# okian/kofft

Measured on AMD Instinct MI355X. Metric: batched 4096-pt c32 FFT throughput, GPoints/s (achieved HBM GB/s: roofline.achieved), higher is better.
Workload: dtype f32

## Files before the change

include/kofft_hip.h:

```cpp
#ifndef KOFFT_HIP_H
#define KOFFT_HIP_H

#include <stddef.h>
#include <stdint.h>

#ifdef __cplusplus
extern "C" {
#endif

#define KOFFT_OK 0
#define KOFFT_ERR_EMPTY_INPUT 1
#define KOFFT_ERR_NON_POWER_OF_TWO_NO_STD 2
#define KOFFT_ERR_MISMATCHED_LENGTHS 3
#define KOFFT_ERR_INVALID_STRIDE 4
#define KOFFT_ERR_INVALID_HOP_SIZE 5
#define KOFFT_ERR_INVALID_VALUE 6
#define KOFFT_ERR_HIP (-1)
#define KOFFT_ERR_UNSUPPORTED (-2)
#define KOFFT_ERR_NULL (-3)
#define KOFFT_ERR_ALLOC (-4)
#define KOFFT_ERR_RCCL (-5)

typedef struct kofft_hip_ctx kofft_hip_ctx;

// ... 198 lines not shown
                                         int mode, float level, int cmap, int depth, int scale, int layout, const uint32_t *pix_of_bin,
                                         void *d_out);
int kofft_hip_set_spectrogram_transpose(kofft_hip_ctx *ctx, int on);
int kofft_hip_stft_picture_f32(kofft_hip_ctx *ctx, const float *signal, size_t rows, size_t len, size_t row_stride, const float *window,
                               size_t win_len, size_t hop, size_t frames, int max_mode, const float *max_in, float *max_out, int mode,
                               float level, int cmap, int depth, int channels, int scale, int layout, const uint32_t *pix_of_bin, void *out);
int kofft_hip_dev_stft_picture_f32(kofft_hip_ctx *ctx, const float *d_signal, size_t rows, size_t len, size_t row_stride,
                                   const float *d_window, size_t win_len, size_t hop, size_t frames, int max_mode, const float *d_max_in,
                                   float *d_max_out, int mode, float level, int cmap, int depth, int channels, int scale, int layout,
                                   const uint32_t *pix_of_bin, void *d_out);
int kofft_hip_log_bin_map(size_t bins, uint32_t *pix_of_bin);
int kofft_hip_map_color_u8(float t, int cmap, unsigned char *rgb);

int kofft_hip_dct_direct_f32(kofft_hip_ctx *ctx, int type, const float *in, float *out, size_t n, size_t batch);
int kofft_hip_dct_direct_f32_dev(kofft_hip_ctx *ctx, int type, const float *d_in, float *d_out, size_t n, size_t batch);
int kofft_hip_dst_direct_f32(kofft_hip_ctx *ctx, int type, const float *in, float *out, size_t n, size_t batch);
int kofft_hip_dst_direct_f32_dev(kofft_hip_ctx *ctx, int type, const float *d_in, float *d_out, size_t n, size_t batch);
int kofft_hip_set_direct_tiled(kofft_hip_ctx *ctx, int on);
int kofft_hip_set_persist_claim_pct(kofft_hip_ctx *ctx, int pct);
int kofft_hip_persist_claim_debug(kofft_hip_ctx *ctx, unsigned out[9]);
int kofft_hip_set_persist_walk(kofft_hip_ctx *ctx, int mode);
int kofft_hip_set_persist_keep_bytes(kofft_hip_ctx *ctx, size_t bytes);
int kofft_hip_persist_walk_debug(kofft_hip_ctx *ctx, unsigned long long out[4]);
int kofft_hip_dct_direct_table_f32(int type, size_t n, float *C);
int kofft_hip_dst_direct_table_f32(int type, size_t n, float *C);
int kofft_hip_dst_planner_table_f32(int type, size_t n, float *out);
int kofft_hip_dst_planner_table_f64(int type, size_t n, double *out);

int kofft_hip_czt_f32(kofft_hip_ctx *ctx, const float *in, float *out, size_t n, size_t m, float wr, float wi, float ar, float ai,
                      size_t batch);
int kofft_hip_dev_czt_f32(kofft_hip_ctx *ctx, const float *d_in, float *d_out, size_t n, size_t m, float wr, float wi, float ar, float ai,
                          size_t batch);
int kofft_hip_goertzel_f32(kofft_hip_ctx *ctx, const float *in, float *out, size_t n, size_t batch, float sample_rate,
                           const float *target_freqs, size_t nfreq);
int kofft_hip_dev_goertzel_f32(kofft_hip_ctx *ctx, const float *d_in, float *d_out, size_t n, size_t batch, float sample_rate,
                               const float *target_freqs, size_t nfreq);
int kofft_hip_set_czt_route(kofft_hip_ctx *ctx, int mode);
int kofft_hip_czt_table_f32(size_t n, size_t m, float wr, float wi, float ar, float ai, float *C);
int kofft_hip_goertzel_coeff_f32(size_t n, float sample_rate, const float *target_freqs, size_t nfreq, float *coeff);

int kofft_hip_dht_f32(kofft_hip_ctx *ctx, const float *in, float *out, size_t n, size_t batch);
int kofft_hip_dev_dht_f32(kofft_hip_ctx *ctx, const float *d_in, float *d_out, size_t n, size_t batch);
int kofft_hip_set_dht_table_device(kofft_hip_ctx *ctx, int on);
int kofft_hip_dht_table_f32(size_t n, float *H);
int kofft_hip_libm_trigf(const float *x, size_t count, float *cos_out, float *sin_out);

// ... 136 lines not shown
```

kofft_amd/_lib.py:

```python
from __future__ import annotations

import ctypes as C
import os
import re
from pathlib import Path

_PKG = Path(__file__).resolve().parent
LIB_PATH = _PKG / "lib" / "libkofft_hip.so"
HEADER_PATH = _PKG.parent / "include" / "kofft_hip.h"


class LibraryMissing(RuntimeError):
    pass


_c_f = C.POINTER(C.c_float)
_c_d = C.POINTER(C.c_double)
_sz = C.c_size_t
_ctx = C.c_void_p

SIGNATURES = {
    "kofft_hip_strerror": (C.c_char_p, [C.c_int]),
    "kofft_hip_last_error": (C.c_char_p, [_ctx]),
    "kofft_hip_version": (C.c_char_p, []),
# ... 105 lines not shown
    "kofft_hip_db_scale_f32": (C.c_int, [_ctx, C.c_void_p, _sz, C.c_void_p, C.c_float, C.c_void_p]),
    "kofft_hip_dev_db_scale_f32": (C.c_int, [_ctx, C.c_void_p, _sz, C.c_void_p, C.c_float, C.c_void_p]),
    "kofft_hip_spectrogram_render_f32": (C.c_int, [_ctx, C.c_void_p, _sz, _sz, C.c_void_p, C.c_int, C.c_float, C.c_int, C.c_int, C.c_int, C.c_int,
                                                   C.c_void_p, C.c_void_p]),
    "kofft_hip_dev_spectrogram_render_f32": (C.c_int, [_ctx, C.c_void_p, _sz, _sz, C.c_void_p, C.c_int, C.c_float, C.c_int, C.c_int, C.c_int, C.c_int,
                                                       C.c_void_p, C.c_void_p]),
    "kofft_hip_set_spectrogram_transpose": (C.c_int, [_ctx, C.c_int]),
    "kofft_hip_stft_picture_f32": (C.c_int, [_ctx, C.c_void_p, _sz, _sz, _sz, C.c_void_p, _sz, _sz, _sz, C.c_int, C.c_void_p, C.c_void_p, C.c_int,
                                             C.c_float, C.c_int, C.c_int, C.c_int, C.c_int, C.c_int, C.c_void_p, C.c_void_p]),
    "kofft_hip_dev_stft_picture_f32": (C.c_int, [_ctx, C.c_void_p, _sz, _sz, _sz, C.c_void_p, _sz, _sz, _sz, C.c_int, C.c_void_p, C.c_void_p, C.c_int,
                                                 C.c_float, C.c_int, C.c_int, C.c_int, C.c_int, C.c_int, C.c_void_p, C.c_void_p]),
    "kofft_hip_log_bin_map": (C.c_int, [_sz, C.c_void_p]),
    "kofft_hip_map_color_u8": (C.c_int, [C.c_float, C.c_int, C.c_void_p]),
    "kofft_hip_dct_direct_f32": (C.c_int, [_ctx, C.c_int, C.c_void_p, C.c_void_p, _sz, _sz]),
    "kofft_hip_dct_direct_f32_dev": (C.c_int, [_ctx, C.c_int, C.c_void_p, C.c_void_p, _sz, _sz]),
    "kofft_hip_dst_direct_f32": (C.c_int, [_ctx, C.c_int, C.c_void_p, C.c_void_p, _sz, _sz]),
    "kofft_hip_dst_direct_f32_dev": (C.c_int, [_ctx, C.c_int, C.c_void_p, C.c_void_p, _sz, _sz]),
    "kofft_hip_set_direct_tiled": (C.c_int, [_ctx, C.c_int]),
    "kofft_hip_set_persist_claim_pct": (C.c_int, [_ctx, C.c_int]),
    "kofft_hip_persist_claim_debug": (C.c_int, [_ctx, C.c_void_p]),
    "kofft_hip_set_persist_walk": (C.c_int, [_ctx, C.c_int]),
    "kofft_hip_set_persist_keep_bytes": (C.c_int, [_ctx, C.c_size_t]),
    "kofft_hip_persist_walk_debug": (C.c_int, [_ctx, C.c_void_p]),
    "kofft_hip_dct_direct_table_f32": (C.c_int, [C.c_int, _sz, C.c_void_p]),
    "kofft_hip_dst_direct_table_f32": (C.c_int, [C.c_int, _sz, C.c_void_p]),
    "kofft_hip_dst_planner_table_f32": (C.c_int, [C.c_int, _sz, C.c_void_p]),
    "kofft_hip_dst_planner_table_f64": (C.c_int, [C.c_int, _sz, C.c_void_p]),
    "kofft_hip_czt_f32": (C.c_int, [_ctx, C.c_void_p, C.c_void_p, _sz, _sz, C.c_float, C.c_float, C.c_float, C.c_float, _sz]),
    "kofft_hip_dev_czt_f32": (C.c_int, [_ctx, C.c_void_p, C.c_void_p, _sz, _sz, C.c_float, C.c_float, C.c_float, C.c_float, _sz]),
    "kofft_hip_goertzel_f32": (C.c_int, [_ctx, C.c_void_p, C.c_void_p, _sz, _sz, C.c_float, C.c_void_p, _sz]),
    "kofft_hip_dev_goertzel_f32": (C.c_int, [_ctx, C.c_void_p, C.c_void_p, _sz, _sz, C.c_float, C.c_void_p, _sz]),
    "kofft_hip_set_czt_route": (C.c_int, [_ctx, C.c_int]),
    "kofft_hip_czt_table_f32": (C.c_int, [_sz, _sz, C.c_float, C.c_float, C.c_float, C.c_float, C.c_void_p]),
    "kofft_hip_dht_f32": (C.c_int, [_ctx, C.c_void_p, C.c_void_p, _sz, _sz]),
    "kofft_hip_dev_dht_f32": (C.c_int, [_ctx, C.c_void_p, C.c_void_p, _sz, _sz]),
    "kofft_hip_set_dht_table_device": (C.c_int, [_ctx, C.c_int]),
    "kofft_hip_dht_table_f32": (C.c_int, [_sz, C.c_void_p]),
    "kofft_hip_libm_trigf": (C.c_int, [C.c_void_p, _sz, C.c_void_p, C.c_void_p]),
    "kofft_hip_window_f32": (C.c_int, [C.c_int, _sz, C.c_float, C.c_void_p]),
    "kofft_hip_goertzel_coeff_f32": (C.c_int, [_sz, C.c_float, C.c_void_p, _sz, C.c_void_p]),
    "kofft_hip_dwt_f32": (C.c_int, [_ctx, C.c_int, C.c_void_p, C.c_void_p, C.c_void_p, _sz, _sz]),
    "kofft_hip_dwt_f32_dev": (C.c_int, [_ctx, C.c_int, C.c_void_p, C.c_void_p, C.c_void_p, _sz, _sz]),
    "kofft_hip_idwt_f32": (C.c_int, [_ctx, C.c_int, C.c_void_p, C.c_void_p, C.c_void_p, _sz, _sz]),
    "kofft_hip_idwt_f32_dev": (C.c_int, [_ctx, C.c_int, C.c_void_p, C.c_void_p, C.c_void_p, _sz, _sz]),
    "kofft_hip_dwt_multi_f32": (C.c_int, [_ctx, C.c_int, C.c_void_p, C.c_void_p, C.c_void_p, _sz, _sz, _sz]),
    "kofft_hip_dwt_multi_f32_dev": (C.c_int, [_ctx, C.c_int, C.c_void_p, C.c_void_p, C.c_void_p, _sz, _sz, _sz]),
# ... 88 lines not shown
```

kofft_amd/api.py:

```python
from __future__ import annotations

import ctypes as C
import os
import enum
from typing import Optional, Sequence

import numpy as np

from . import _lib


class FftError(Exception):

    EmptyInput = 1
    NonPowerOfTwoNoStd = 2
    MismatchedLengths = 3
    InvalidStride = 4
    InvalidHopSize = 5
    InvalidValue = 6
    _names = {1: "EmptyInput", 2: "NonPowerOfTwoNoStd", 3: "MismatchedLengths", 4: "InvalidStride",
              5: "InvalidHopSize", 6: "InvalidValue"}

    def __init__(self, code: int):
        self.code = int(code)
# ... 993 lines not shown
            raise TypeError("the Hartley transform is f32-only, like the reference (hartley.rs)")
        a = self._rbuf(x)
        if a.ndim != 2:
            raise TypeError("dht_batch expects a 2-D [batch, n] array")
        out = np.empty(a.shape, np.float32)
        self._check(self._lib.kofft_hip_dht_f32(self._ctx, _ptr(a), _ptr(out), a.shape[1], a.shape[0]))
        return out

    def dht_dev(self, d_in: int, d_out: int, n: int, batch: int) -> None:
        if min(int(n), int(batch)) < 0:
            raise ValueError("n and batch are usize in the reference: they cannot be negative")
        self._check(self._lib.kofft_hip_dev_dht_f32(self._ctx, C.c_void_p(d_in), C.c_void_p(d_out), int(n), int(batch)))

    def set_dht_table_device(self, on: bool) -> None:
        self._check(self._lib.kofft_hip_set_dht_table_device(self._ctx, int(bool(on))))

    def set_persist_claim_pct(self, pct: int) -> None:
        self._check(self._lib.kofft_hip_set_persist_claim_pct(self._ctx, int(pct)))

    def set_persist_walk(self, mode: int, keep_bytes: int | None = None) -> None:
        self._check(self._lib.kofft_hip_set_persist_walk(self._ctx, int(mode)))
        if keep_bytes is not None:
            self._check(self._lib.kofft_hip_set_persist_keep_bytes(self._ctx, int(keep_bytes)))

    def set_czt_route(self, mode: int) -> None:
        self._check(self._lib.kofft_hip_set_czt_route(self._ctx, int(mode)))

    def _spectral_in(self, x, what: str):
        if self.dtype != np.float32:
            raise TypeError(f"{what} is f32-only, like the reference ({what}.rs)")
        dev = hasattr(x, "data_ptr") and hasattr(x, "is_cuda")
        if dev:
            import torch

            if not x.is_cuda or x.dtype != torch.float32:
                raise TypeError(f"{what}: a torch input must be a float32 tensor on the device")
            a = x.contiguous()
        else:
            a = np.ascontiguousarray(x, np.float32)
        if a.ndim not in (1, 2):
            raise TypeError(f"{what} expects a 1-D signal or a 2-D [batch, n] array")
        return (a.reshape(1, -1) if a.ndim == 1 else a), a.ndim == 1, dev

    def czt(self, x, m: int, w, a):
        rows, one, dev = self._spectral_in(x, "czt")
        if int(m) < 0:
# ... 1302 lines not shown
```

kofft_amd/csrc/fft_persist.hip.h:

```cpp
#pragma once

#include "fft_wg.hip.h"

namespace kofft {

template <typename T, int L, int S0, int Q>
__device__ __forceinline__ void load_pass_twiddles(cpx<T> *twr, const int k, const cpx<T> *__restrict__ tw)
{
#pragma unroll
    for (int t = 0; t < Q; ++t) {
#pragma unroll
        for (int h = 0; h < (1 << t); ++h) {
            const int idx = (k << (L - 1 - S0 - t)) + (bitrev(h, t) << (L - 1 - t));
            twr[(1 << t) - 1 + h] = tw[idx];
        }
    }
}

template <typename T, int Q>
__device__ __forceinline__ void reg_pass_r(cpx<T> *v, const cpx<T> *twr)
{
#pragma unroll
    for (int t = 0; t < Q; ++t) {
        const int pos = Q - 1 - t;
// ... 82 lines not shown
template <class CFG, class = void>
struct persist_depth { static constexpr int value = 1; };
template <class CFG>
struct persist_depth<CFG, decltype((void)CFG::DEPTH)> { static constexpr int value = CFG::DEPTH; };

template <class CFG, class = void>
struct persist_tw_global { static constexpr bool value = false; };
template <class CFG>
struct persist_tw_global<CFG, decltype((void)CFG::kTwGlobal)> { static constexpr bool value = CFG::kTwGlobal; };

template <class CFG, class = void>
struct persist_claim { static constexpr bool value = false; };
template <class CFG>
struct persist_claim<CFG, decltype((void)CFG::kClaim)> { static constexpr bool value = CFG::kClaim; };

constexpr unsigned kPersistClaimShards = 2, kPersistClaimMaxShards = 8, kPersistClaimLine = 128 / sizeof(unsigned);
static_assert(kPersistClaimShards >= 1 && kPersistClaimShards <= kPersistClaimMaxShards, "claim words");
constexpr size_t kPersistClaimBytes = (kPersistClaimMaxShards + 1) * 128;
struct PersistClaim {
    unsigned *counters;
    size_t split;
    size_t keep_from;
    unsigned mirror;
};
constexpr unsigned long long kPersistClaimEmpty = ~0ull;
template <class IO>
struct PersistClaimIO : IO {
    PersistClaim claim;
};
struct NoXchg {
    static constexpr bool keep = false;
    __device__ __forceinline__ void put() const {}
    __device__ __forceinline__ void get() const {}
};

template <typename T, int L, int RL, int EPI, class IO, class CFG>
struct PersistState {
    static constexpr int R = 1 << RL;
    static constexpr int NP = (L + RL - 1) / RL;
    static constexpr bool TWG = persist_tw_global<CFG>::value;
    static constexpr bool TW1_REG = !TWG && !(NP == 2 && CFG::kTwLastInLds);
    static constexpr bool TW2_REG = !TWG && NP >= 3 && !(CFG::kTwLastInLds && NP == 3);
    static constexpr bool TW3_REG = !TWG && NP >= 4 && !CFG::kTwLastInLds;
    cpx<T> tw1[TW1_REG ? R - 1 : 1], tw2[TW2_REG ? R - 1 : 1], tw3[TW3_REG ? R - 1 : 1];
    typename IO::Inv inv[CFG::kInvInLds ? 1 : R];
    const typename IO::Inv *inv_lds;
    const cpx<T> *tw_lds;
    const cpx<T> *rt_lds;
    int g1, g2, g3, sc;
};

template <class IO, int TPT, bool PAIR = io_pairs_in_wave<IO>::value>
struct persist_raw {
    using type = typename IO::Raw;
    static constexpr int extra = 0;
    static constexpr bool pair = false, pair_lds = false;
};
// ... 178 lines not shown
            constexpr int NK = R / 2;
            cpx<T> kept[NK];
            int ki = 0;
#pragma unroll
            for (int u = 0; u < R; ++u)
                if (LastG::out_index(0, u) < N / 2) kept[ki++] = cur[u];
            float m[NK];
            const float top = IO::template mags_of<NK>(kept, m);
            ki = 0;
#pragma unroll
            for (int u = 0; u < R; ++u)
                if (LastG::out_index(0, u) < N / 2) io.store_d_mag(od, lane_bytes, LastG::out_index(0, u), m[ki++], row_off);
            if constexpr (io_row_acc<IO>::value) io.acc_row(xf0, active ? top : 0.0f);
            else if (active) acc = __builtin_fmaxf(acc, top);
        } else if constexpr (io_half_keep<IO>::value) {
            static_assert((LastG::out_index(0, 1) % TPT) == 0 && TPT <= N / 2, "register part and thread part of the index: disjoint bit fields");
#pragma unroll
            for (int u = 0; u < R; ++u) {
                if (LastG::out_index(0, u) < N / 2) io.store_d_kept(od, lane_bytes, LastG::out_index(0, u), cur[u], row_off);
                else if (LastG::out_index(0, u) == N / 2) io.store_d_nyquist(od, tau, LastG::out_index(0, u), cur[u], row_off);
            }
        } else {
        if constexpr (persist_claim<CFG>::value) {
            if (xchg.keep) {
#pragma unroll
                for (int u = 0; u < R; ++u) io.template store_d<AUX_DEFAULT>(od, lane_bytes, LastG::out_index(0, u), cur[u], row_off);
            } else {
#pragma unroll
                for (int u = 0; u < R; ++u) io.template store_d<kStoreAux>(od, lane_bytes, LastG::out_index(0, u), cur[u], row_off);
            }
        } else {
#pragma unroll
        for (int u = 0; u < R; ++u) {
            if constexpr (io_has_acc<IO>::value) io.store_d_acc(od, lane_bytes, LastG::out_index(0, u), cur[u], row_off, acc);
            else io.store_d(od, lane_bytes, LastG::out_index(0, u), cur[u], row_off);
        }
        }
        }
    }
}

template <typename T, int L, int RL, int EPI, class IO, class CFG>
__global__ __launch_bounds__(CFG::BLOCK, CFG::MINW) void fft_persist_kernel(const IO io, const cpx<T> *__restrict__ tw,
                                                                            const size_t batch)
{
    constexpr int BLOCK = CFG::BLOCK, NBUF = CFG::NBUF;
    constexpr int N = 1 << L;
// ... 126 lines not shown
        return;
    }

    constexpr int DEPTH = persist_depth<CFG>::value;
    static_assert(DEPTH == 1 || DEPTH == 2, "prefetch distance");
    Raw ra[RS], rb[RS];
    const int in_lane_bytes = tau * IO::kRawBytes;
    const int in_row_off = (G == 1) ? 0 : sub * (int)io.in_slot_bytes();
    auto group_cnt = [&](size_t b) -> int {
        const size_t first = b + wslot;
        return first >= batch ? 0 : (batch - first < (size_t)G ? (int)(batch - first) : G);
    };
    auto issue = [&](Raw *dst, const size_t b) {
        const rsrc_t d = io.in_desc_n(mem_row(b) + wslot, group_cnt(b));
        if constexpr (RawSel::pair || RawSel::pair_lds) {
#pragma unroll
            for (int u = 0; u < R; ++u) dst[u] = io.fetch_pair_d(d, in_lane_bytes, FirstG::in_index(0, u), in_row_off);
            dst[R] = io.fetch_last_d(d, in_row_off);
        } else {
#pragma unroll
            for (int u = 0; u < R; ++u) dst[u] = io.fetch_d(d, in_lane_bytes, FirstG::in_index(0, u), in_row_off);
        }
    };
    issue(ra, base);
    typename persist_acc<IO>::type acc{};
    if constexpr (io_has_acc<IO>::value) acc = io.acc_init();
    auto finish = [&]() {
        if constexpr (io_has_acc<IO>::value) io.acc_finish(acc);
        if constexpr (CLAIMS) claim_leave();
    };

    if constexpr (CLAIMS) {
        struct ClaimXchg {
            unsigned long long *word;
            size_t first;
            unsigned len;
            const unsigned *ticket;
            size_t *claimed;
            bool writer;
            bool keep;
            __device__ __forceinline__ void put() const
            {
                if (writer) {
                    const unsigned off = XPB * *ticket;
                    *word = off < len ? first + off : kPersistClaimEmpty;
                }
            }
            __device__ __forceinline__ void get() const { *claimed = *word; }
        };
        auto claim_walk_on = [&]() -> size_t {
            if (tid == 0) {
                ++claim_exhausted;
                claim_shard = (claim_shard + 1) % kPersistClaimShards;
                claim_word[1] = claim_now();
            }
            __syncthreads();
            return claim_word[1];
        };
#define KOFFT_PERSIST_STEP_CLAIM(CUR, NXT, LEAVE)                                                                    \
    {                                                                                                                \
        const bool more = nbase < batch;                                                      \
        const bool walked = nbase + step < io.claim.split;                                    \
        const bool claims = more && !walked && tid == 0;                                                             \
        unsigned ticket;  \
        size_t claimed = batch;                                                                                      \
        if (claims) ticket = atomicAdd(claim_counter(claim_shard), 1u);                                              \
        __builtin_amdgcn_sched_barrier(0);                                   \
        issue(NXT, nbase);                                                                                           \
        __builtin_amdgcn_sched_barrier(0);                           \
        const ClaimXchg xchg{claim_word, io.claim.split + (size_t)claim_shard * claim_piece, claim_len(claim_shard), &ticket, &claimed, claims, \
                             __builtin_amdgcn_readfirstlane((unsigned)(base >= io.claim.keep_from)) != 0u}; \
        persist_transform<T, L, RL, EPI, CFG>(CUR, st, io, tw, buf0, buf1, mem_row(base) + wslot, group_cnt(base), sub, tau, acc, NoPrefetchParts{}, xchg); \
        if (!more) LEAVE;                                                                                            \
         \
        if (!walked && __builtin_amdgcn_readfirstlane((unsigned)(claimed >> 32)) == ~0u) claimed = claim_walk_on();   \
        base = nbase;                                                                                                \
        nbase = walked ? nbase + step : (size_t)claimed;                         \
    }
        KOFFT_PERSIST_STEP_CLAIM(ra, rb, { finish(); return; })
        for (;;) {
            KOFFT_PERSIST_STEP_CLAIM(rb, ra, break)
            KOFFT_PERSIST_STEP_CLAIM(ra, rb, break)
        }
        finish();
#undef KOFFT_PERSIST_STEP_CLAIM
    } else if constexpr (DEPTH == 1 && St::TWG && !(RawSel::pair || RawSel::pair_lds)) {
        constexpr bool TOP = persist_twg_top_part(L);
        constexpr int PARTS = TOP ? NP : NP - 1;
#define KOFFT_PERSIST_STEP_PARTS(CUR, NXT, LEAVE)                                                                    \
    {                                                                                                                \
        const size_t nbase = base + step;                                                                            \
        const bool more = nbase < batch;                                                      \
        const rsrc_t nd = io.in_desc_n(nbase + wslot, group_cnt(nbase));                                             \
        auto part = [&](const int i) {                                                                               \
            _Pragma("unroll") for (int u = 0; u < R; ++u)                                                            \
                if (u * PARTS / R == i) NXT[u] = io.fetch_d(nd, in_lane_bytes, FirstG::in_index(0, u), in_row_off);  \
        };                                                                                                           \
        if constexpr (TOP) {                                                                                         \
            part(0);                                                                                                 \
            __builtin_amdgcn_sched_barrier(0);                                                                       \
        }                                                                                                            \
        persist_transform<T, L, RL, EPI, CFG>(CUR, st, io, tw, buf0, buf1, base + wslot, group_cnt(base), sub, tau, acc, part); \
        if (!more) LEAVE;                                                                                            \
        base = nbase;                                                                                                \
    }
        KOFFT_PERSIST_STEP_PARTS(ra, rb, { finish(); return; })
        for (;;) {
// ... 49 lines not shown
```

kofft_amd/csrc/fft_wg.hip.h:

```cpp
#pragma once

#include "fft_device.hip.h"

namespace kofft {

__host__ __device__ constexpr int lds_pad(int i) { return i + (i >> 4); }
__host__ __device__ constexpr int lds_elems(int n) { return n + (n >> 4) + 1; }


struct NoInv {};

template <class IO, class = void>
struct io_has_acc { static constexpr bool value = false; };
template <class IO>
struct io_has_acc<IO, decltype((void)IO::kHasAcc)> { static constexpr bool value = IO::kHasAcc; };
template <class IO, class = void>
struct io_frame_rem { static constexpr bool value = false; };
template <class IO>
struct io_frame_rem<IO, decltype((void)IO::kFrameRem)> { static constexpr bool value = IO::kFrameRem; };
template <class IO, class = void>
struct io_half_spectrum { static constexpr bool value = false; };
template <class IO>
struct io_half_spectrum<IO, decltype((void)IO::kHalfSpectrum)> { static constexpr bool value = IO::kHalfSpectrum; };

// ... 38 lines not shown
    __device__ __forceinline__ Raw fetch(size_t xf, int i) const { return ld_stream(in + xf * (size_t)n + i); }
    static constexpr int kRawBytes = sizeof(cpx<T>);
    __device__ __forceinline__ rsrc_t in_desc(size_t xf, bool valid) const
    {
        return make_rsrc(in + (valid ? xf : 0) * (size_t)n, valid ? (unsigned)n * sizeof(cpx<T>) : 0u);
    }
    __device__ __forceinline__ rsrc_t out_desc(size_t xf) const { return make_rsrc(out + xf * (size_t)n, (unsigned)n * sizeof(cpx<T>)); }
    __device__ __forceinline__ rsrc_t in_desc_n(size_t xf0, int cnt) const
    {
        return make_rsrc(in + (cnt > 0 ? xf0 : 0) * (size_t)n, (unsigned)(cnt > 0 ? cnt : 0) * (unsigned)n * (unsigned)sizeof(cpx<T>));
    }
    __device__ __forceinline__ rsrc_t out_desc_n(size_t xf0, int cnt) const
    {
        return make_rsrc(out + (cnt > 0 ? xf0 : 0) * (size_t)n, (unsigned)(cnt > 0 ? cnt : 0) * (unsigned)n * (unsigned)sizeof(cpx<T>));
    }
    __device__ __forceinline__ unsigned out_row_bytes() const { return (unsigned)n * sizeof(cpx<T>); }
    __device__ __forceinline__ bool wg_desc_ok(int) const { return true; }
    __device__ __forceinline__ unsigned in_slot_bytes() const { return (unsigned)n * sizeof(cpx<T>); }
    __device__ __forceinline__ rsrc_t in_desc_wg(size_t xf0, size_t batch, int xpb) const
    {
        const size_t cnt = xf0 < batch ? (batch - xf0 < (size_t)xpb ? batch - xf0 : (size_t)xpb) : 0;
        return make_rsrc(in + (cnt ? xf0 : 0) * (size_t)n, (unsigned)(cnt * n * sizeof(cpx<T>)));
    }
    __device__ __forceinline__ Raw fetch_d(rsrc_t d, int lane_bytes, int iu, int row_off = 0) const
    {
        return buf_load_cpx<T, kCLoadAux>(d, row_off + lane_bytes, iu * (int)sizeof(cpx<T>));
    }
    template <int AUX = kStoreAux>
    __device__ __forceinline__ void store_d(rsrc_t d, int lane_bytes, int ou, cpx<T> v, int row_off = 0) const
    {
        if (INVERSE) {
            const T im = -v.im;
            v.re = v.re * scale;
            v.im = im * scale;
        }
        if constexpr (AUX == kStoreAux) buf_store_cpx<T>(v, d, row_off + lane_bytes, ou * (int)sizeof(cpx<T>));
        else buf_store_cpx_aux<T, AUX>(v, d, row_off + lane_bytes, ou * (int)sizeof(cpx<T>));
    }
    __device__ __forceinline__ Inv invariant(int) const { return {}; }
    __device__ __forceinline__ cpx<T> finish(size_t, int, Raw v, Inv) const
    {
        if (INVERSE) v.im = -v.im;
        return v;
    }
    __device__ __forceinline__ bool inside(size_t) const { return true; }
    __device__ __forceinline__ cpx<T> finish_in(Raw v, Inv w) const { return finish(0, 0, v, w); }
    __device__ __forceinline__ cpx<T> load(size_t xf, int i) const { return finish(xf, i, fetch(xf, i), {}); }
    __device__ __forceinline__ void store(size_t xf, int o, cpx<T> v) const
    {
// ... 1007 lines not shown
```

kofft_amd/csrc/host_common.hip.h:

```cpp
#pragma once

#include "../../include/kofft_hip.h"

#include <hip/hip_runtime.h>

#include <atomic>
#include <climits>
#include <cstdio>
#include <cstdlib>
#include <cstring>
#include <map>
#include <new>
#include <string>
#include <utility>
#include <vector>

#include "fft_big.hip.h"
#include "fft_persist.hip.h"
#include "fft_istft.hip.h"
#include "fft_regfile.hip.h"
#include "fft_split_wide.hip.h"
#include "fft_wg.hip.h"
#include "host_cache.h"
#include "host_layout.h"
// ... 36 lines not shown
    bool convolve_bank_fused = true;
    bool mdct_fused = true;
    int pfb_fused = 1;
    int mfcc_fused = 1;
    int frontend_fused = 1;
    int welch_fused = 1;
    int resample_tiled = 1;
    int sosfilt_tiled = 1;
    bool spec_transpose = true;
    bool direct_tiled = true;
    bool dht_table_device = true;
    int wavelet_fused = 1;
    int czt_route = 0;
    bool blue_persist = true;
    int persist_grid_pct = 0;
    int persist_claim_pct = -1;
    unsigned *persist_claim_counters = nullptr;
    int persist_walk_mode = kofft::host::kPersistWalkRule;
    size_t persist_keep_bytes = kofft::host::kPersistKeepDefaultBytes;
    kofft::host::PersistWalkRecord persist_walk_last;
    unsigned long long persist_walk_launches = 0;
    kofft::host::PersistWalkPlan persist_walk_plan_last{false, 0};
    size_t persist_walk_batch_last = 0;
    int big_three_min = 22;
    bool small32 = true;
    bool big_first11 = true;
    bool big_narrow = true;
    bool big_persist = true;
    bool blue_fused = true;
    bool blue_one_kernel = true;
    bool nd_transpose = true;
    bool nd_fused = true;
    bool nd_two_pass = true;
    bool zero_copy = true;
    bool host_pipeline = true;
    bool rfft14_wide = true;
    bool rfft13_persist = true;
    int persist64 = 1;
    bool persist_small = true;
    bool rfft_regfile_epi = true;
    bool use_regfile = true;
    bool use_split = true;
    std::string last_error;
    kofft::host::TableCache tables;
    std::vector<kofft_spectral_slot> czt_slots;
    void *goertzel_coeff = nullptr;
// ... 310 lines not shown

template <typename T, int L, int EPI, class IO>
int launch_persist_claim(kofft_hip_ctx *ctx, const IO &io, const cpx<T> *tw, size_t batch);
template <typename T, int L, int EPI, class IO>
int launch_persist(kofft_hip_ctx *ctx, const IO &io, const cpx<T> *tw, size_t batch)
{
    using Cfg = PersistCfg<L, IO>;
    if constexpr (persist_claim<Cfg>::value) return launch_persist_claim<T, L, EPI>(ctx, io, tw, batch);
    else {
    constexpr int RL = Cfg::RL;
    constexpr int XPB = Cfg::BLOCK / ((1 << L) >> RL);
    constexpr size_t lds = (size_t)XPB * Cfg::NBUF * persist_slot_elems(L) * sizeof(cpx<T>) +
                           (Cfg::kInvInLds ? (size_t)(1 << L) * sizeof(typename IO::Inv) : 0) +
                           (EPI == EPI_RFFT ? (size_t)(1 << L) * sizeof(cpx<T>) : 0) +
                           (Cfg::kTwLastInLds ? (size_t)(1 << L) / 2 * sizeof(cpx<T>) : 0);
    static_assert(lds * Cfg::WG_PER_CU <= 160 * 1024, "LDS budget");
    static std::atomic<unsigned long long> attr_done{0};
    const size_t blocks = resident_blocks(ctx->num_cus, PersistGrid<L, IO>::wg_per_cu(Cfg::WG_PER_CU, batch * sizeof(cpx<T>) << L),
                                          ctx->persist_grid_pct, (batch + XPB - 1) / XPB);
    return launch_resident(ctx, attr_done, fft_persist_kernel<T, L, RL, EPI, IO, Cfg>, blocks, Cfg::BLOCK, lds, io, tw, batch);
    }
}

template <typename T, int L, int EPI, class IO>
int launch_persist_claim(kofft_hip_ctx *ctx, const IO &io, const cpx<T> *tw, size_t batch)
{
    using Cfg = PersistCfg<L, IO>;
    constexpr int RL = Cfg::RL;
    constexpr int XPB = Cfg::BLOCK / ((1 << L) >> RL);
    constexpr size_t lds = (size_t)XPB * Cfg::NBUF * persist_slot_elems(L) * sizeof(cpx<T>) + 16;
    static_assert(lds * Cfg::WG_PER_CU <= 160 * 1024, "LDS budget");
    if (!ctx->persist_claim_counters) {
        ctx->last_error = "the context has no claim counters";
        return KOFFT_ERR_ALLOC;
    }
    using KIO = PersistClaimIO<IO>;
    static std::atomic<unsigned long long> attr_done{0};
    const size_t blocks = resident_blocks(ctx->num_cus, PersistGrid<L, IO>::wg_per_cu(Cfg::WG_PER_CU, batch * sizeof(cpx<T>) << L),
                                          ctx->persist_grid_pct, (batch + XPB - 1) / XPB);
    const size_t stride = blocks * XPB;
    const size_t pct = ctx->persist_claim_pct < 0 ? (size_t)Cfg::kClaimPct : (ctx->persist_claim_pct > 100 ? 100 : (size_t)ctx->persist_claim_pct);
    size_t claimed = batch / 100 * pct + batch % 100 * pct / 100;
    if (claimed > (size_t(1) << 31)) claimed = size_t(1) << 31;
    const size_t row_bytes = sizeof(cpx<T>) << L, bytes = batch * row_bytes;
    const uintptr_t in_lo = reinterpret_cast<uintptr_t>(io.in), out_lo = reinterpret_cast<uintptr_t>(io.out);
    const kofft::host::PersistWalkPlan plan = kofft::host::persist_walk_plan(ctx->persist_walk_mode, ctx->persist_walk_last, in_lo, bytes, out_lo,
                                                                             bytes, batch, row_bytes, ctx->persist_keep_bytes);
    ctx->persist_walk_last = kofft::host::PersistWalkRecord{out_lo, bytes, plan.mirror};
    ctx->persist_walk_plan_last = plan;
    ctx->persist_walk_batch_last = batch;
    ++ctx->persist_walk_launches;
    const KIO kio{io, PersistClaim{ctx->persist_claim_counters, (batch - claimed) / stride * stride, plan.keep_from, plan.mirror ? 1u : 0u}};
    return launch_resident(ctx, attr_done, fft_persist_kernel<T, L, RL, EPI, KIO, Cfg>, blocks, Cfg::BLOCK, lds, kio, tw, batch);
}

template <typename T, int LA, int LB, class IO>
int launch_split(kofft_hip_ctx *ctx, const IO &io, const cpx<T> *tw, size_t batch)
{
    using Gm = SplitGeom<LA, LB>;
    constexpr size_t lds = 2 * (size_t)Gm::N * sizeof(cpx<T>) + 16;
    static_assert(lds <= 160 * 1024, "LDS budget");
    static std::atomic<unsigned long long> attr_done{0};
    const size_t blocks = resident_blocks(ctx->num_cus, 1, ctx->persist_grid_pct, batch);
    return launch_resident(ctx, attr_done, fft_split_persist_kernel<T, LA, LB, IO>, blocks, Gm::TPT, lds, io, tw, batch);
}


template <typename T, int LA, int LB, int QB0, class IO>
int launch_split_wide(kofft_hip_ctx *ctx, const IO &io, const cpx<T> *tw, size_t batch)
{
    using Gm = SplitWideGeom<LA, LB, QB0>;
    constexpr size_t lds = split_wide_lds_bytes<Gm>();
    static_assert(lds <= 160 * 1024, "LDS budget");
    static std::atomic<unsigned long long> attr_done{0};
    const size_t blocks = resident_blocks(ctx->num_cus, (int)((160 * 1024) / lds), ctx->persist_grid_pct, batch);
    return launch_resident(ctx, attr_done, fft_split_wide_persist_kernel<T, LA, LB, QB0, IO>, blocks, Gm::TPT, lds, io, tw, batch);
// ... 220 lines not shown
```

kofft_amd/csrc/kofft_hip.hip:

```cpp
#include "host_stage.hip.h"

#include <condition_variable>
#include <mutex>
#include <thread>

namespace kofft {
namespace host {

int pipeline_chunks(kofft_hip_ctx *ctx, size_t nchunks, const std::function<hipError_t(size_t, hipStream_t)> &up,
                    const std::function<int(size_t)> &run, const std::function<hipError_t(size_t, hipStream_t)> &down)
{
    hipStream_t s_in = nullptr, s_out = nullptr;
    std::vector<hipEvent_t> uploaded(nchunks, nullptr), done(nchunks, nullptr);
    auto cleanup = [&]() {
        for (size_t c = 0; c < nchunks; ++c) {
            if (uploaded[c]) (void)hipEventDestroy(uploaded[c]);
            if (done[c]) (void)hipEventDestroy(done[c]);
        }
        if (s_in) (void)hipStreamDestroy(s_in);
        if (s_out) (void)hipStreamDestroy(s_out);
    };
    bool ok = hipStreamCreateWithFlags(&s_in, hipStreamNonBlocking) == hipSuccess &&
              hipStreamCreateWithFlags(&s_out, hipStreamNonBlocking) == hipSuccess;
    for (size_t c = 0; c < nchunks && ok; ++c)
// ... 296 lines not shown
    if (!ctx->persist_claim_counters) return KOFFT_ERR_ALLOC;
    KOFFT_HIP_TRY(ctx, hipSetDevice(ctx->device));
    KOFFT_HIP_TRY(ctx, hipStreamSynchronize(ctx->stream));
    for (unsigned s = 0; s <= kofft::kPersistClaimMaxShards; ++s)
        KOFFT_HIP_TRY(ctx, hipMemcpy(out + s, ctx->persist_claim_counters + s * kofft::kPersistClaimLine, sizeof(unsigned), hipMemcpyDeviceToHost));
    return KOFFT_OK;
}
int kofft_hip_set_persist_walk(kofft_hip_ctx *ctx, int mode) { return set_route(ctx, &kofft_hip_ctx::persist_walk_mode, mode, -1, 2); }
int kofft_hip_set_persist_keep_bytes(kofft_hip_ctx *ctx, size_t bytes)
{
    if (!ctx) return KOFFT_ERR_NULL;
    ctx->persist_keep_bytes = bytes;
    return KOFFT_OK;
}
int kofft_hip_persist_walk_debug(kofft_hip_ctx *ctx, unsigned long long out[4])
{
    if (!ctx || !out) return KOFFT_ERR_NULL;
    out[0] = ctx->persist_walk_launches;
    out[1] = ctx->persist_walk_plan_last.mirror ? 1u : 0u;
    out[2] = ctx->persist_walk_plan_last.keep_from;
    out[3] = ctx->persist_walk_batch_last;
    return KOFFT_OK;
}

}
```

kofft_amd/csrc/persist_walk.h:

```cpp
#pragma once
#include <cstddef>
#include <cstdint>

namespace kofft {
namespace host {

struct PersistWalkRecord {
    uintptr_t lo = 0;
    size_t bytes = 0;
    bool mirrored = false;
};

enum : int { kPersistWalkRule = -1, kPersistWalkParent = 0, kPersistWalkAscKeep = 1, kPersistWalkDescKeep = 2 };
constexpr size_t kPersistKeepDefaultBytes = size_t(256) << 20;

inline bool persist_walk_is(const PersistWalkRecord &r, uintptr_t p, size_t bytes) { return r.bytes != 0 && r.lo == p && r.bytes == bytes; }

inline bool persist_walk_rule(const PersistWalkRecord &r, uintptr_t in, size_t in_bytes, uintptr_t out, size_t out_bytes)
{
    return (persist_walk_is(r, in, in_bytes) || persist_walk_is(r, out, out_bytes)) ? !r.mirrored : false;
}

inline size_t persist_keep_from(size_t batch, size_t row_bytes, size_t keep_bytes, bool clamp)
{
    if (row_bytes == 0 || batch == 0) return batch;
    const size_t rows = keep_bytes / row_bytes;
    if (rows == 0) return batch;
    if (clamp) return rows >= batch ? 0 : batch - rows;
    return rows > batch / 2 ? batch : batch - rows;
}

inline size_t persist_mem_row(size_t batch, size_t w, bool mirror) { return mirror ? batch - 1 - w : w; }

struct PersistWalkPlan {
    bool mirror;
    size_t keep_from;
};

inline PersistWalkPlan persist_walk_plan(int mode, const PersistWalkRecord &r, uintptr_t in, size_t in_bytes, uintptr_t out, size_t out_bytes,
                                         size_t batch, size_t row_bytes, size_t keep_bytes)
{
    switch (mode) {
    case kPersistWalkParent: return {false, batch};
    case kPersistWalkAscKeep: return {false, persist_keep_from(batch, row_bytes, keep_bytes, true)};
    case kPersistWalkDescKeep: return {true, persist_keep_from(batch, row_bytes, keep_bytes, true)};
    default: return {persist_walk_rule(r, in, in_bytes, out, out_bytes), persist_keep_from(batch, row_bytes, keep_bytes, false)};
    }
}

}
}
```

Baseline: 410.9.

## Use cache-resident load/store hints for head rows kept from previous launch

Adds a head-step phase to the claim-based persistent FFT kernel. For the rows the previous launch left cache-resident (tracked via kept_rows in the walk record), loads use default cache aux bits instead of streaming, and stores always use the keep path. The kernel is templated on a HEAD policy with four instantiations, and the loop prologue is restructured to run head_steps iterations before the normal streaming loop. This adds code-size and template complexity, and the gain depends on whether the previous output really is still in cache.

```diff
diff --git a/include/kofft_hip.h b/include/kofft_hip.h
--- a/include/kofft_hip.h
+++ b/include/kofft_hip.h
@@ -244,6 +244,8 @@
 int kofft_hip_set_persist_walk(kofft_hip_ctx *ctx, int mode);
 int kofft_hip_set_persist_keep_bytes(kofft_hip_ctx *ctx, size_t bytes);
 int kofft_hip_persist_walk_debug(kofft_hip_ctx *ctx, unsigned long long out[4]);
+int kofft_hip_set_persist_head(kofft_hip_ctx *ctx, int policy);
+int kofft_hip_persist_head_debug(kofft_hip_ctx *ctx, unsigned long long out[3]);
 int kofft_hip_dct_direct_table_f32(int type, size_t n, float *C);
 int kofft_hip_dst_direct_table_f32(int type, size_t n, float *C);
 int kofft_hip_dst_planner_table_f32(int type, size_t n, float *out);
diff --git a/kofft_amd/_lib.py b/kofft_amd/_lib.py
--- a/kofft_amd/_lib.py
+++ b/kofft_amd/_lib.py
@@ -151,6 +151,8 @@
     "kofft_hip_set_persist_walk": (C.c_int, [_ctx, C.c_int]),
     "kofft_hip_set_persist_keep_bytes": (C.c_int, [_ctx, C.c_size_t]),
     "kofft_hip_persist_walk_debug": (C.c_int, [_ctx, C.c_void_p]),
+    "kofft_hip_set_persist_head": (C.c_int, [_ctx, C.c_int]),
+    "kofft_hip_persist_head_debug": (C.c_int, [_ctx, C.c_void_p]),
     "kofft_hip_dct_direct_table_f32": (C.c_int, [C.c_int, _sz, C.c_void_p]),
     "kofft_hip_dst_direct_table_f32": (C.c_int, [C.c_int, _sz, C.c_void_p]),
     "kofft_hip_dst_planner_table_f32": (C.c_int, [C.c_int, _sz, C.c_void_p]),
diff --git a/kofft_amd/api.py b/kofft_amd/api.py
--- a/kofft_amd/api.py
+++ b/kofft_amd/api.py
@@ -1039,6 +1039,14 @@
         self._check(self._lib.kofft_hip_set_persist_walk(self._ctx, int(mode)))
         if keep_bytes is not None:
             self._check(self._lib.kofft_hip_set_persist_keep_bytes(self._ctx, int(keep_bytes)))
+
+    def set_persist_head(self, policy: int) -> None:
+        self._check(self._lib.kofft_hip_set_persist_head(self._ctx, int(policy)))
+
+    def persist_head_debug(self) -> tuple[int, bool, bool]:
+        words = (C.c_ulonglong * 3)()
+        self._check(self._lib.kofft_hip_persist_head_debug(self._ctx, words))
+        return int(words[0]), bool(words[1]), bool(words[2])
 
     def set_czt_route(self, mode: int) -> None:
         self._check(self._lib.kofft_hip_set_czt_route(self._ctx, int(mode)))
diff --git a/kofft_amd/csrc/fft_persist.hip.h b/kofft_amd/csrc/fft_persist.hip.h
--- a/kofft_amd/csrc/fft_persist.hip.h
+++ b/kofft_amd/csrc/fft_persist.hip.h
@@ -128,10 +128,12 @@
     size_t split;
     size_t keep_from;
     unsigned mirror;
+    unsigned head_steps;
 };
 constexpr unsigned long long kPersistClaimEmpty = ~0ull;
-template <class IO>
+template <class IO, int HEAD = 0>
 struct PersistClaimIO : IO {
+    static constexpr int kHead = HEAD;
     PersistClaim claim;
 };
 struct NoXchg {
@@ -139,6 +141,10 @@
     __device__ __forceinline__ void put() const {}
     __device__ __forceinline__ void get() const {}
 };
+template <class X, class = void>
+struct xchg_keeps_all { static constexpr bool value = false; };
+template <class X>
+struct xchg_keeps_all<X, std::void_t<typename X::keeps_all>> { static constexpr bool value = true; };
 
 template <typename T, int L, int RL, int EPI, class IO, class CFG>
 struct PersistState {
@@ -363,7 +369,10 @@
             }
         } else {
         if constexpr (persist_claim<CFG>::value) {
-            if (xchg.keep) {
+            if constexpr (xchg_keeps_all<Xchg>::value) {
+#pragma unroll
+                for (int u = 0; u < R; ++u) io.template store_d<AUX_DEFAULT>(od, lane_bytes, LastG::out_index(0, u), cur[u], row_off);
+            } else if (xchg.keep) {
 #pragma unroll
                 for (int u = 0; u < R; ++u) io.template store_d<AUX_DEFAULT>(od, lane_bytes, LastG::out_index(0, u), cur[u], row_off);
             } else {
@@ -536,7 +545,7 @@
             for (int u = 0; u < R; ++u) dst[u] = io.fetch_d(d, in_lane_bytes, FirstG::in_index(0, u), in_row_off);
         }
     };
-    issue(ra, base);
+    if constexpr (!CLAIMS) issue(ra, base);
     typename persist_acc<IO>::type acc{};
     if constexpr (io_has_acc<IO>::value) acc = io.acc_init();
     auto finish = [&]() {
@@ -571,7 +580,19 @@
             __syncthreads();
             return claim_word[1];
         };
-#define KOFFT_PERSIST_STEP_CLAIM(CUR, NXT, LEAVE)                                                                    \
+        struct ClaimXchgKept : ClaimXchg {
+            using keeps_all [[maybe_unused]] = void;
+        };
+        constexpr int kHeadLoadAux = (IO::kHead & 1) ? AUX_DEFAULT : kCLoadAux;
+        using HeadXchg = std::conditional_t<(IO::kHead & 2) != 0, ClaimXchgKept, ClaimXchg>;
+        auto issue_aux = [&](auto aux, Raw *dst, const size_t b) {
+            const rsrc_t d = io.in_desc_n(mem_row(b) + wslot, group_cnt(b));
+#pragma unroll
+            for (int u = 0; u < R; ++u) dst[u] = io.template fetch_d<decltype(aux)::value>(d, in_lane_bytes, FirstG::in_index(0, u), in_row_off);
+        };
+        using StreamAux = std::integral_constant<int, kCLoadAux>;
+        using HeadAux = std::integral_constant<int, kHeadLoadAux>;
+#define KOFFT_PERSIST_STEP_CLAIM(CUR, NXT, LEAVE, ISSUE, XCHG)                                                       \
     {                                                                                                                \
         const bool more = nbase < batch;                                                      \
         const bool walked = nbase + step < io.claim.split;                                    \
@@ -580,10 +601,10 @@
         size_t claimed = batch;                                                                                      \
         if (claims) ticket = atomicAdd(claim_counter(claim_shard), 1u);                                              \
         __builtin_amdgcn_sched_barrier(0);                                   \
-        issue(NXT, nbase);                                                                                           \
+        ISSUE;                                                           \
         __builtin_amdgcn_sched_barrier(0);                           \
-        const ClaimXchg xchg{claim_word, io.claim.split + (size_t)claim_shard * claim_piece, claim_len(claim_shard), &ticket, &claimed, claims, \
-                             __builtin_amdgcn_readfirstlane((unsigned)(base >= io.claim.keep_from)) != 0u}; \
+        const XCHG xchg{ClaimXchg{claim_word, io.claim.split + (size_t)claim_shard * claim_piece, claim_len(claim_shard), &ticket, &claimed, claims, \
+                             __builtin_amdgcn_readfirstlane((unsigned)(base >= io.claim.keep_from)) != 0u}}; \
         persist_transform<T, L, RL, EPI, CFG>(CUR, st, io, tw, buf0, buf1, mem_row(base) + wslot, group_cnt(base), sub, tau, acc, NoPrefetchParts{}, xchg); \
         if (!more) LEAVE;                                                                                            \
          \
@@ -591,12 +612,37 @@
         base = nbase;                                                                                                \
         nbase = walked ? nbase + step : (size_t)claimed;                         \
     }
-        KOFFT_PERSIST_STEP_CLAIM(ra, rb, { finish(); return; })
+#define KOFFT_PERSIST_LEAVE { finish(); return; }
+        unsigned head_steps = io.claim.head_steps;
+        if (head_steps == 0) {
+            issue_aux(StreamAux{}, ra, base);
+        } else {
+            if (head_steps & 1) {
+                issue_aux(HeadAux{}, rb, base);
+                KOFFT_PERSIST_STEP_CLAIM(rb, ra, KOFFT_PERSIST_LEAVE,
+                                         if (head_steps == 1) issue_aux(StreamAux{}, ra, nbase); else issue_aux(HeadAux{}, ra, nbase), HeadXchg)
+                --head_steps;
+            } else {
+                issue_aux(HeadAux{}, ra, base);
+            }
+            if (head_steps != 0) {
+                KOFFT_PERSIST_STEP_CLAIM(ra, rb, KOFFT_PERSIST_LEAVE, issue_aux(HeadAux{}, rb, nbase), HeadXchg)
+                if (unsigned pairs = (head_steps - 2) / 2) {
+                    do {
+                        KOFFT_PERSIST_STEP_CLAIM(rb, ra, KOFFT_PERSIST_LEAVE, issue_aux(HeadAux{}, ra, nbase), HeadXchg)
+                        KOFFT_PERSIST_STEP_CLAIM(ra, rb, KOFFT_PERSIST_LEAVE, issue_aux(HeadAux{}, rb, nbase), HeadXchg)
+                    } while (--pairs != 0);
+                }
+                KOFFT_PERSIST_STEP_CLAIM(rb, ra, KOFFT_PERSIST_LEAVE, issue_aux(StreamAux{}, ra, nbase), HeadXchg)
+            }
+        }
+        KOFFT_PERSIST_STEP_CLAIM(ra, rb, KOFFT_PERSIST_LEAVE, issue_aux(StreamAux{}, rb, nbase), ClaimXchg)
         for (;;) {
-            KOFFT_PERSIST_STEP_CLAIM(rb, ra, break)
-            KOFFT_PERSIST_STEP_CLAIM(ra, rb, break)
+            KOFFT_PERSIST_STEP_CLAIM(rb, ra, break, issue_aux(StreamAux{}, ra, nbase), ClaimXchg)
+            KOFFT_PERSIST_STEP_CLAIM(ra, rb, break, issue_aux(StreamAux{}, rb, nbase), ClaimXchg)
         }
         finish();
+#undef KOFFT_PERSIST_LEAVE
 #undef KOFFT_PERSIST_STEP_CLAIM
     } else if constexpr (DEPTH == 1 && St::TWG && !(RawSel::pair || RawSel::pair_lds)) {
         constexpr bool TOP = persist_twg_top_part(L);
diff --git a/kofft_amd/csrc/fft_wg.hip.h b/kofft_amd/csrc/fft_wg.hip.h
--- a/kofft_amd/csrc/fft_wg.hip.h
+++ b/kofft_amd/csrc/fft_wg.hip.h
@@ -84,9 +84,10 @@
         const size_t cnt = xf0 < batch ? (batch - xf0 < (size_t)xpb ? batch - xf0 : (size_t)xpb) : 0;
         return make_rsrc(in + (cnt ? xf0 : 0) * (size_t)n, (unsigned)(cnt * n * sizeof(cpx<T>)));
     }
+    template <int AUX = kCLoadAux>
     __device__ __forceinline__ Raw fetch_d(rsrc_t d, int lane_bytes, int iu, int row_off = 0) const
     {
-        return buf_load_cpx<T, kCLoadAux>(d, row_off + lane_bytes, iu * (int)sizeof(cpx<T>));
+        return buf_load_cpx<T, AUX>(d, row_off + lane_bytes, iu * (int)sizeof(cpx<T>));
     }
     template <int AUX = kStoreAux>
     __device__ __forceinline__ void store_d(rsrc_t d, int lane_bytes, int ou, cpx<T> v, int row_off = 0) const
diff --git a/kofft_amd/csrc/host_common.hip.h b/kofft_amd/csrc/host_common.hip.h
--- a/kofft_amd/csrc/host_common.hip.h
+++ b/kofft_amd/csrc/host_common.hip.h
@@ -82,6 +82,8 @@
     unsigned long long persist_walk_launches = 0;
     kofft::host::PersistWalkPlan persist_walk_plan_last{false, 0};
     size_t persist_walk_batch_last = 0;
+    int persist_head_policy = kofft::host::kPersistHeadDefault;
+    kofft::host::PersistHeadPlan persist_head_plan_last{0, false, false};
     int big_three_min = 22;
     bool small32 = true;
     bool big_first11 = true;
@@ -438,6 +440,16 @@
     }
 }
 
+template <typename T, int L, int EPI, int HEAD, class IO>
+int launch_persist_claim_head(kofft_hip_ctx *ctx, const IO &io, const PersistClaim &claim, size_t blocks, size_t lds, const cpx<T> *tw, size_t batch)
+{
+    using Cfg = PersistCfg<L, IO>;
+    using KIO = PersistClaimIO<IO, HEAD>;
+    static std::atomic<unsigned long long> attr_done{0};
+    const KIO kio{io, claim};
+    return launch_resident(ctx, attr_done, fft_persist_kernel<T, L, Cfg::RL, EPI, KIO, Cfg>, blocks, Cfg::BLOCK, lds, kio, tw, batch);
+}
+
 template <typename T, int L, int EPI, class IO>
 int launch_persist_claim(kofft_hip_ctx *ctx, const IO &io, const cpx<T> *tw, size_t batch)
 {
@@ -450,8 +462,6 @@
         ctx->last_error = "the context has no claim counters";
         return KOFFT_ERR_ALLOC;
     }
-    using KIO = PersistClaimIO<IO>;
-    static std::atomic<unsigned long long> attr_done{0};
     const size_t blocks = resident_blocks(ctx->num_cus, PersistGrid<L, IO>::wg_per_cu(Cfg::WG_PER_CU, batch * sizeof(cpx<T>) << L),
                                           ctx->persist_grid_pct, (batch + XPB - 1) / XPB);
     const size_t stride = blocks * XPB;
@@ -462,12 +472,21 @@
     const uintptr_t in_lo = reinterpret_cast<uintptr_t>(io.in), out_lo = reinterpret_cast<uintptr_t>(io.out);
     const kofft::host::PersistWalkPlan plan = kofft::host::persist_walk_plan(ctx->persist_walk_mode, ctx->persist_walk_last, in_lo, bytes, out_lo,
                                                                              bytes, batch, row_bytes, ctx->persist_keep_bytes);
-    ctx->persist_walk_last = kofft::host::PersistWalkRecord{out_lo, bytes, plan.mirror};
+    const size_t split = (batch - claimed) / stride * stride;
+    const kofft::host::PersistHeadPlan head = kofft::host::persist_head_plan(ctx->persist_walk_mode, ctx->persist_walk_last, in_lo, bytes, out_lo, bytes,
+                                                                             batch, row_bytes, ctx->persist_keep_bytes, split, stride, ctx->persist_head_policy);
+    ctx->persist_walk_last = kofft::host::PersistWalkRecord{out_lo, bytes, plan.mirror, batch - plan.keep_from};
     ctx->persist_walk_plan_last = plan;
+    ctx->persist_head_plan_last = head;
     ctx->persist_walk_batch_last = batch;
     ++ctx->persist_walk_launches;
-    const KIO kio{io, PersistClaim{ctx->persist_claim_counters, (batch - claimed) / stride * stride, plan.keep_from, plan.mirror ? 1u : 0u}};
-    return launch_resident(ctx, attr_done, fft_persist_kernel<T, L, RL, EPI, KIO, Cfg>, blocks, Cfg::BLOCK, lds, kio, tw, batch);
+    const PersistClaim claim{ctx->persist_claim_counters, split, plan.keep_from, plan.mirror ? 1u : 0u, (unsigned)(head.head_to / stride)};
+    switch ((head.loads ? 1 : 0) | (head.stores ? 2 : 0)) {
+    case 1: return launch_persist_claim_head<T, L, EPI, 1>(ctx, io, claim, blocks, lds, tw, batch);
+    case 2: return launch_persist_claim_head<T, L, EPI, 2>(ctx, io, claim, blocks, lds, tw, batch);
+    case 3: return launch_persist_claim_head<T, L, EPI, 3>(ctx, io, claim, blocks, lds, tw, batch);
+    default: return launch_persist_claim_head<T, L, EPI, 0>(ctx, io, claim, blocks, lds, tw, batch);
+    }
 }
 
 template <typename T, int LA, int LB, class IO>
diff --git a/kofft_amd/csrc/kofft_hip.hip b/kofft_amd/csrc/kofft_hip.hip
--- a/kofft_amd/csrc/kofft_hip.hip
+++ b/kofft_amd/csrc/kofft_hip.hip
@@ -342,5 +342,14 @@
     out[3] = ctx->persist_walk_batch_last;
     return KOFFT_OK;
 }
-
-}
+int kofft_hip_set_persist_head(kofft_hip_ctx *ctx, int policy) { return set_route(ctx, &kofft_hip_ctx::persist_head_policy, policy, 0, 3); }
+int kofft_hip_persist_head_debug(kofft_hip_ctx *ctx, unsigned long long out[3])
+{
+    if (!ctx || !out) return KOFFT_ERR_NULL;
+    out[0] = ctx->persist_head_plan_last.head_to;
+    out[1] = ctx->persist_head_plan_last.loads ? 1u : 0u;
+    out[2] = ctx->persist_head_plan_last.stores ? 1u : 0u;
+    return KOFFT_OK;
+}
+
+}
diff --git a/kofft_amd/csrc/persist_walk.h b/kofft_amd/csrc/persist_walk.h
--- a/kofft_amd/csrc/persist_walk.h
+++ b/kofft_amd/csrc/persist_walk.h
@@ -9,6 +9,7 @@
     uintptr_t lo = 0;
     size_t bytes = 0;
     bool mirrored = false;
+    size_t kept_rows = 0;
 };
 
 enum : int { kPersistWalkRule = -1, kPersistWalkParent = 0, kPersistWalkAscKeep = 1, kPersistWalkDescKeep = 2 };
@@ -48,5 +49,37 @@
     }
 }
 
+enum : int { kPersistHeadNone = 0, kPersistHeadLoads = 1, kPersistHeadStores = 2, kPersistHeadBoth = 3 };
+constexpr int kPersistHeadDefault = kPersistHeadBoth;
+struct PersistHeadPlan {
+    size_t head_to;
+    bool loads, stores;
+};
+
+inline PersistHeadPlan persist_head_plan(int mode, const PersistWalkRecord &r, uintptr_t in, size_t in_bytes, uintptr_t out, size_t out_bytes,
+                                         size_t batch, size_t row_bytes, size_t keep_bytes, size_t split, size_t stride, int policy)
+{
+    size_t rows = 0;
+    bool in_match = false, out_match = false;
+    switch (mode) {
+    case kPersistWalkParent: break;
+    case kPersistWalkAscKeep:
+    case kPersistWalkDescKeep:
+        rows = batch - persist_keep_from(batch, row_bytes, keep_bytes, true);
+        in_match = out_match = true;
+        break;
+    default:
+        in_match = persist_walk_is(r, in, in_bytes);
+        out_match = persist_walk_is(r, out, out_bytes);
+        if (in_match || out_match) rows = r.kept_rows;
+        break;
+    }
+    if (rows > batch) rows = batch;
+    if (rows > split) rows = split;
+    const size_t head_to = stride == 0 ? 0 : rows / stride * stride;
+    if (head_to == 0) return {0, false, false};
+    return {head_to, in_match && (policy & kPersistHeadLoads) != 0, out_match && (policy & kPersistHeadStores) != 0};
+}
+
 }
 }
```

Result: no change. 410.0 (-0.2%).
